# octaviogarcia/RaytracingOneWeekend

Hardware: AMD Instinct MI355X
Metric: Msamples/s (W×H×spp/s) + achieved HBM GB/s, 1080p@512spp traced scene (higher is better)
Workload: dtype f32; 1 GPU; C1 S-traced 1920x1080, 10496 spp timed (128 spp/step), depth 50; width=1920, height=1080, max_depth=50, parallelism=tile1, gather=RCCL send/recv (om_gather_frame), rccl_library=/usr/local/lib/python3.10/dist-packages/torch/lib/librccl.so, kernel=auto, pipeline=auto, tail_bounce=default, streams=2

## Files before the change

raytracingoneweekend_amd/csrc/om_tuning.h:

```cpp
#pragma once

#ifndef OM_WF_BLOCK
#define OM_WF_BLOCK 512
#endif
#ifndef OM_WF_WAVES
#define OM_WF_WAVES 8
#endif
#ifndef OM_WF_TAIL_SPB
#define OM_WF_TAIL_SPB 2
#endif
#ifndef OM_WF_TAIL_WGS_PER_CU
#define OM_WF_TAIL_WGS_PER_CU 1
#endif
#ifndef OM_WF_MAX_PATHS_LOG2
#define OM_WF_MAX_PATHS_LOG2 27
#endif
#ifndef OM_WF_BATCH_SPP
#define OM_WF_BATCH_SPP 16
#endif
#ifndef OM_WF_MIN_PATHS_LOG2
#define OM_WF_MIN_PATHS_LOG2 25
#endif
#ifndef OM_WF_HYB_BYTES
#define OM_WF_HYB_BYTES 16384
#endif
#ifndef OM_WF_HYBW_BYTES
#define OM_WF_HYBW_BYTES 0
#endif
#ifndef OM_WF_HYB4_BYTES
#define OM_WF_HYB4_BYTES 0
#endif
#ifndef OM_WF_REFILL
#define OM_WF_REFILL 16
#endif
#ifndef OM_WF_TAIL_SHADE
#define OM_WF_TAIL_SHADE 1
#endif
#ifndef OM_WF_TAIL_UNROLL
#define OM_WF_TAIL_UNROLL 24
#endif
#ifndef OM_WF_TAIL_MARCH_WAVES
#define OM_WF_TAIL_MARCH_WAVES 8
#endif
#ifndef OM_WF_TAIL_REFILL
#define OM_WF_TAIL_REFILL OM_WF_REFILL
#endif
#ifndef OM_WF_TAIL_MARCHED
#define OM_WF_TAIL_MARCHED 1
#endif
#ifndef OM_MARCH_UNROLL
#define OM_MARCH_UNROLL 8
#endif
#ifndef OM_WF_ADAPTIVE_BATCHES
#define OM_WF_ADAPTIVE_BATCHES 3
#endif
#ifndef OM_WF_ADAPTIVE_PATHS_LOG2
#define OM_WF_ADAPTIVE_PATHS_LOG2 22
#endif
#ifndef OM_WF_ADAPTIVE_CAP_LOG2
#define OM_WF_ADAPTIVE_CAP_LOG2 26
#endif
#ifndef OM_WF_ADAPTIVE_TAIL
#define OM_WF_ADAPTIVE_TAIL 8
#endif
#ifndef OM_WF_LANES_PER_CU
#define OM_WF_LANES_PER_CU 2048
#endif
#ifndef OM_WF_LANES_PER_CU_WIDE
#define OM_WF_LANES_PER_CU_WIDE 8192
#endif
#ifndef OM_WF_DEAL_BLOCKS
#define OM_WF_DEAL_BLOCKS 8
#endif
#ifndef OM_ACC_GROUP
#define OM_ACC_GROUP 8
#endif
#ifndef OM_B2_NODE_STRIDE
#define OM_B2_NODE_STRIDE 80
#endif
#ifndef OM_BARY_TREE_MIN
#define OM_BARY_TREE_MIN 16
#endif
```

raytracingoneweekend_amd/csrc/om_wavefront.hip:

```cpp
#include "om_wavefront.h"

#include <algorithm>
#include <type_traits>

#include "om_device.h"
#include "om_trace.h"
#include "om_tuning.h"
#include "om_deal.h"

using namespace omd;

namespace omw {

void QueueSet::release() {
    for (int a = 0; a < 2; ++a) {
        for (int b = 0; b < 3; ++b) { if (q[a][b]) (void)hipFree(q[a][b]); q[a][b] = nullptr; }
        if (qr[a]) (void)hipFree(qr[a]); qr[a] = nullptr;
    }
    if (res) (void)hipFree(res);
    if (res_id) (void)hipFree(res_id);
    if (counts) (void)hipFree(counts);
    if (hit) (void)hipFree(hit);
    res = nullptr; res_id = nullptr; counts = nullptr; hit = nullptr;
}

void Buffers::release() {
    for (auto& s : set) s.release();
    if (n0) (void)hipFree(n0);
    n0 = nullptr; n0_cap = 0;
    for (auto& st : side) { if (st) (void)hipStreamDestroy(st); st = nullptr; }

    for (auto e : ev) (void)hipEventDestroy(e);
    ev.clear();
    cap = 0; counts_n = 0; nsets = 0;
}

namespace {

constexpr uint32_t kNoSample = 0xFFFFFFFFu;
enum { TR_BRUTE = 1, TR_CULLED = 2, TR_BVH = 3, TR_SBVH_LDS = 4, TR_SBVH_GLOBAL = 5, TR_BVH2_LDS = 6, TR_BVH2_GLOBAL = 7,
       TR_BVH4_LDS = 8, TR_BVH4_GLOBAL = 9,
       TR_BVH2_WIDE = 10,
       TR_BARY = 16 };
constexpr int tr_base(int tr) { return tr & (TR_BARY - 1); }
constexpr bool tr_bary(int tr) { return (tr & TR_BARY) != 0; }
#define OM_WAVES_ATTR __attribute__((amdgpu_waves_per_eu(OM_WF_WAVES, OM_WF_WAVES)))
constexpr int kBlk = OM_WF_BLOCK;
constexpr int kStackDepth = 24;
constexpr uint32_t kB2Stride = OM_B2_NODE_STRIDE;
static_assert(kB2Stride % 16u == 0u && kB2Stride >= sizeof(OmBvh2Node), "16-B aligned node slots");
static_assert(kB2LdsBudget / sizeof(OmBvh2Node) * (kB2Stride / 16u) < OM_LEAF, "scaled BVH2 child codes stay below OM_LEAF");
template <int TR>
__host__ __device__ inline uint32_t stack_bytes(const OmSceneDev& S) {
    if (tr_base(TR) == TR_BVH2_WIDE) return kBlk * S.b2w_stack * 4u;
    return kBlk * ((tr_base(TR) == TR_BVH4_LDS || tr_base(TR) == TR_BVH4_GLOBAL) ? S.b4_stack : S.b2_stack) * 2u;
}
__host__ __device__ inline uint32_t b2_stage_bytes(const OmSceneDev& S) {
    return (S.n_b2nodes * kB2Stride + S.n_b2leaves * 4u + 15u) & ~15u;
}
constexpr uint32_t kTailSpb = OM_WF_TAIL_SPB;
constexpr uint32_t kTailWgsPerCu = OM_WF_TAIL_WGS_PER_CU;
constexpr uint32_t kWaves = kBlk / 64;
static_assert(kBlk % 64 == 0 && kTailWgsPerCu >= 1u, "whole waves; a tail grid");
constexpr uint32_t kTailDefault = 16;
constexpr uint32_t kTailMarched = OM_WF_TAIL_MARCHED;
constexpr uint32_t kTailL2 = 10;
constexpr uint32_t kTailBigBatch = 24;
__host__ __device__ inline uint32_t hyb_nodes(const OmSceneDev& S) {
    constexpr uint32_t kCap = OM_WF_HYB_BYTES / (uint32_t)sizeof(OmBvh2NodeH);
    return S.b2_lds_bytes ? 0u : (S.n_b2nodes < kCap ? S.n_b2nodes : kCap);
}
static_assert(sizeof(OmBvh2NodeW) == sizeof(OmBvh2NodeH), "wide and half nodes share a buffer");
__host__ __device__ inline const OmBvh2NodeW* wide_nodes(const OmSceneDev& S) { return (const OmBvh2NodeW*)(S.b2h + S.n_b2nodes); }
__host__ __device__ inline uint32_t hybw_nodes(const OmSceneDev& S) {
    constexpr uint32_t kCap = OM_WF_HYBW_BYTES / (uint32_t)sizeof(OmBvh2NodeW);
    return S.n_b2wnodes < kCap ? S.n_b2wnodes : kCap;
}
__host__ __device__ inline uint32_t hyb4_nodes(const OmSceneDev& S) {
    constexpr uint32_t kCap = OM_WF_HYB4_BYTES / (uint32_t)sizeof(OmBvh4NodeH);
    return S.b4_lds_bytes ? 0u : (S.n_b4nodes < kCap ? S.n_b4nodes : kCap);
}
using MarchedC2Lds = MarchedExactLds<2, 1, 1>;
enum { MV_ARRAYS = 0, MV_EXACT_C2_LDS = 1 };
template <int TR>
__host__ __device__ constexpr bool exact_view_built() { return TR == TR_BRUTE || TR == TR_BVH2_LDS; }
__host__ __device__ inline Deal batch_deal(uint64_t paths, uint32_t nseg) { return make_deal(paths, nseg, OM_WF_DEAL_BLOCKS); }

extern __shared__ __attribute__((aligned(16))) uint4 wf_lds[];

__device__ __forceinline__ uint32_t wave_sum32(uint32_t v) {
#pragma unroll
    for (int off = 32; off > 0; off >>= 1) v += __shfl_xor(v, off, 64);
    return v;
}
__device__ __forceinline__ void flush_counter(unsigned long long* ctr, int slot, uint32_t v) {
    v = wave_sum32(v);
    if (__lane_id() == 0 && v) atomicAdd(&ctr[slot], (unsigned long long)v);
}

struct Seg {
    uint32_t nseg;
    uint32_t segcap;
};

struct AdPlan { uint32_t c, done; };
struct AdCfg {
    uint32_t sample_count;
    uint32_t batches;
    uint32_t paths;
};
__host__ __device__ inline uint32_t ad_batch(uint32_t c, uint32_t done, uint32_t j, const AdCfg& A) {
    if (c == 0u || done >= A.sample_count || j >= A.batches) return 0u;
    const uint32_t rem = A.sample_count - done, left = A.batches - j;
    const uint32_t even = (rem + left - 1u) / left, want = A.paths / c;
    const uint32_t b = even > want ? even : want;
    return b < rem ? b : rem;
}
struct AdList {
    const uint32_t* list;
    const AdPlan* plan;
    uint32_t* list_next;
    AdPlan* plan_next;
    AdCfg A;
    uint32_t j;
};

struct Queue {
    float4* q0; float4* q1; float4* q2; uint4* qr;
};

struct Gen {
    OmCamDev C;
    const float2* jitter;
    const om_pixel_stats* stats;
    const uint32_t* pixels;
    uint32_t n_pixels, by_pixel, batch;
    const uint32_t* n0;
    uint32_t done;
    AdList ad;
    const uint32_t* tile_off;
    const uint16_t* tile_idx;
    const float* tile_tnear;
};

struct Path {
    F3 o, d, cur;
// ... 123 lines not shown
                                     float& closest, Wk& w) {
    closest = P.tmax;
    int best = trace_traced<TR>(S, T, o, d, P.tmin, closest, w);
    if (MARCH) {
        float tm;
        const int mg = march(S, o, d, P.tmin, P.tmax, closest, P.march_steps, tm, w);
        if (mg >= 0) { best = mg; closest = tm; }
    }
    return best;
}

template <bool MARCH, bool USER = MARCH>
__device__ __forceinline__ bool shade_path(const OmSceneDev& S, const OmParamsDev& P, uint32_t depth_cap, Path& p,
                                           float closest, int best, float4* __restrict__ res,
                                           uint32_t* __restrict__ res_id) {
    float seg_depth; uint32_t seg_id;
    if (best >= 0) {
        F3 point, normal;
        finalize<MARCH, USER>(S, best, p.o, p.d, P.tmin, closest, point, normal);
        F3 nd, att;
        scatter(S.mats[best], p.d, normal, p.g, nd, att);
        p.cur = mul(p.cur, att);
        p.o = point; p.d = unit(nd);
        seg_depth = closest; seg_id = (uint32_t)best + 1u;
    } else {
        const float t = 0.5f * (p.d.y + 1.0f);
        p.cur = mul(p.cur, f3((1.0f - t) + 0.5f * t, (1.0f - t) + 0.7f * t, (1.0f - t) + 1.0f * t));
        seg_depth = INFINITY; seg_id = 0u;
    }
    bool finished = false;
    F3 result = p.cur;
    float rdepth = 0.0f; uint32_t rid = 0;
    if (p.seg == 0u) {
        p.depthf = seg_depth; p.first_id = seg_id;
        if (isinf(seg_depth)) { finished = true; rdepth = INFINITY; rid = 0u; }
    } else if (isinf(seg_depth)) {
        finished = true; rdepth = p.depthf; rid = p.first_id;
    }
    if (!finished && p.seg + 1u >= depth_cap) {
        finished = true; result = f3(-0.0f, -0.0f, -0.0f); rdepth = p.depthf; rid = p.first_id;
    }
    if (finished) {
        res[p.slot] = make_float4(result.x, result.y, result.z, rdepth);
        res_id[p.slot] = rid;
        return false;
    }
    p.seg += 1u;
    return true;
}

__device__ __forceinline__ bool gen_path(const OmParamsDev& P, const Gen& R, uint32_t stride, uint64_t i, Path& p,
                                         uint32_t& pixel, uint32_t* __restrict__ res_id) {
    const uint32_t s_local = (uint32_t)i / stride, kk = (uint32_t)i - s_local * stride;
    const uint32_t k = R.ad.list ? R.ad.list[kk] : kk;
    pixel = R.pixels[k];
    uint32_t s;
    bool live;
    if (R.n0) {
        const uint32_t v = R.n0[k];
        s = (v & 0x7FFFFFFFu) + R.done + s_local;
        live = s < P.spp_total && !(v >> 31);
    } else {
        const om_pixel_stats& ps = R.stats[R.by_pixel ? pixel : k];
        s = ps.n + s_local;
        live = s < P.spp_total && !(P.adaptive && (ps.flags & 1u));
    }
    if (!live) {
        res_id[i] = kNoSample;
        return false;
    }
    p.g = path_rng(P.skey, pixel, s);
    const uint32_t line = pixel / P.width;
    gen_camera_ray(R.C, P, R.jitter, (float)(pixel - P.width * line), (float)line, s, p.g, p.o, p.d);
    p.cur = f3(1.0f, 1.0f, 1.0f); p.depthf = 0.0f; p.first_id = 0u; p.seg = 0u; p.slot = (uint32_t)i;
    return true;
}

template <int TR, bool COUNT, bool MARCH, bool FIRST, bool HIT = false, bool USER = MARCH>
__global__ __launch_bounds__(kBlk) OM_WAVES_ATTR void k_bounce(OmSceneDev S, OmParamsDev P, Seg G, Gen R, Queue in,
                                                 const uint32_t* __restrict__ count_in, Queue out,
                                                 uint32_t* __restrict__ count_out, float4* __restrict__ res,
                                                 uint32_t* __restrict__ res_id, unsigned long long* __restrict__ counters,
                                                 const float2* __restrict__ hitbuf, uint32_t* __restrict__ tail_next) {
    const uint64_t seg0 = (uint64_t)blockIdx.x * G.segcap;
    uint32_t n, stride = R.n_pixels;
    Deal dl{};
    if (FIRST) {
        if (tail_next && blockIdx.x == 0 && threadIdx.x == 0) *tail_next = 0u;
        uint64_t paths = (uint64_t)R.n_pixels * R.batch;
        if (R.ad.list) {
            const AdPlan pl = uniform_load(R.ad.plan);
            stride = pl.c;
            paths = (uint64_t)pl.c * ad_batch(pl.c, pl.done, R.ad.j, R.ad.A);
        }
        dl = batch_deal(paths, G.nseg);
        n = dl.blocks_of(blockIdx.x);
    } else {
        n = count_in[blockIdx.x];
    }
    if (n == 0) {
        if (threadIdx.x == 0) count_out[blockIdx.x] = 0u;
        return;
    }
    __shared__ uint32_t q_next, q_out;
    if (threadIdx.x == 0) { q_next = kBlk / 64u; q_out = 0u; }
    __syncthreads();
    const Tracer T = HIT ? Tracer{} : stage_scene<TR>(S);
    const uint32_t depth_cap = P.max_depth > 1u ? P.max_depth : 1u;
    WorkT<COUNT, false, tr_bary(TR)> w;
    uint32_t segs = 0;
    const uint32_t lane = __lane_id();
    const uint32_t chunks = FIRST ? n : (n + 63u) / 64u;
    for (uint32_t chunk = __builtin_amdgcn_readfirstlane(threadIdx.x >> 6); chunk < chunks;) {
        const uint64_t i = FIRST ? dl.block(blockIdx.x, chunk) * 64u + lane : seg0 + chunk * 64u + lane;
        bool keep = false;
        Path p;
        uint32_t p_pixel = 0;
        if (FIRST ? i < dl.paths : chunk * 64u + lane < n) {
            bool live = true;
            if (FIRST) {
                live = gen_path(P, R, stride, i, p, p_pixel, res_id);
            } else {
                load_ray(in, i, p);
                load_rest(in, i, p);
            }
            if (live) {
                float closest;
                int best;
                if (HIT) {
                    const float2 h = hitbuf[i];
                    closest = h.x; best = __float_as_int(h.y);
                } else if (FIRST && (tr_base(TR) == TR_BVH2_LDS || tr_base(TR) == TR_BVH2_GLOBAL || tr_base(TR) == TR_BVH2_WIDE) && R.tile_off) {
                    const uint32_t line = p_pixel / P.width;
                    const uint32_t tile = (p_pixel - line * P.width) / 8u + (line / 8u) * P.tiles_x;
                    closest = P.tmax;
                    const uint32_t t0 = __builtin_amdgcn_readfirstlane(tile);
                    if (__ballot(tile != t0) == 0)
                        best = traced_tiles<true>(S, R.tile_off, R.tile_idx, t0, p.o, p.d, P.tmin, closest, w, R.tile_tnear);
                    else
                        best = traced_tiles(S, R.tile_off, R.tile_idx, tile, p.o, p.d, P.tmin, closest, w);
                    if (MARCH) {
                        float tm;
                        const int mg = march(S, p.o, p.d, P.tmin, P.tmax, closest, P.march_steps, tm, w);
                        if (mg >= 0) { best = mg; closest = tm; }
                    }
                } else {
                    best = trace<TR, MARCH>(S, P, T, p.o, p.d, closest, w);
                }
                keep = shade_path<MARCH, USER>(S, P, depth_cap, p, closest, best, res, res_id);
                if (COUNT) segs++;
            }
        }
        const uint64_t m = __ballot(keep);
        uint32_t obase = 0u, nc = 0u;
        if (lane == 0) {
            obase = m ? atomicAdd(&q_out, (uint32_t)__popcll(m)) : 0u;
            nc = atomicAdd(&q_next, 1u);
        }
        obase = __builtin_amdgcn_readfirstlane(obase);
        chunk = __builtin_amdgcn_readfirstlane(nc);
        if (keep) store_path(out, seg0 + obase + (uint32_t)__popcll(m & ((1ull << lane) - 1ull)), p);
    }
    __syncthreads();
    if (threadIdx.x == 0) count_out[blockIdx.x] = q_out;
    if (COUNT) {
        flush_counter(counters, OMC_SEGMENTS, segs);
        flush_counter(counters, OMC_PRIM_TESTS, w.prim);
        flush_counter(counters, OMC_PRE_TESTS, w.pre);
        flush_counter(counters, OMC_MARCH, w.march);
    }
}

template <bool COUNT>
__global__ __launch_bounds__(kBlk) OM_WAVES_ATTR void k_raygen(OmParamsDev P, Seg G, Gen R, Queue out,
                                                 uint32_t* __restrict__ count_out, uint32_t* __restrict__ res_id) {
    const uint64_t seg0 = (uint64_t)blockIdx.x * G.segcap;
    uint64_t paths = (uint64_t)R.n_pixels * R.batch;
    uint32_t stride = R.n_pixels;
    if (R.ad.list) {
        const AdPlan pl = uniform_load(R.ad.plan);
        stride = pl.c;
        paths = (uint64_t)pl.c * ad_batch(pl.c, pl.done, R.ad.j, R.ad.A);
    }
    const Deal dl = batch_deal(paths, G.nseg);
    const uint32_t nblk = dl.blocks_of(blockIdx.x);
    __shared__ uint32_t q_out;
    if (threadIdx.x == 0) q_out = 0u;
    __syncthreads();
    const uint32_t lane = __lane_id();
    for (uint32_t c = threadIdx.x >> 6; c < nblk; c += kBlk / 64u) {
        const uint64_t i = dl.block(blockIdx.x, c) * 64u + lane;
        Path p;
        uint32_t pixel;
        const bool keep = i < dl.paths && gen_path(P, R, stride, i, p, pixel, res_id);
        const uint64_t m = __ballot(keep);
        uint32_t obase = 0u;
        if (lane == 0 && m) obase = atomicAdd(&q_out, (uint32_t)__popcll(m));
        obase = __builtin_amdgcn_readfirstlane(obase);
        if (keep) store_path(out, seg0 + obase + (uint32_t)__popcll(m & ((1ull << lane) - 1ull)), p);
    }
    __syncthreads();
    if (threadIdx.x == 0) count_out[blockIdx.x] = q_out;
}

template <int TR, bool COUNT, class M, class Wk>
__device__ __forceinline__ void march_lanes(const OmSceneDev& S, const OmParamsDev& P, const Tracer& T, const M& m,
                                            const Queue& in, uint64_t seg0, uint32_t n, uint32_t& next,
                                            float2* __restrict__ hit, Wk& w) {
    const uint32_t lane = __lane_id();
    uint32_t j = threadIdx.x;
    bool act = j < n, marching = false;
    bool dry = !act;
    F3 o = f3(0.0f, 0.0f, 0.0f), d = o;
    float t = 0.0f, closest = 0.0f;
    int best = -1;
    uint32_t iters = 0;
    auto start = [&]() {
        const float4 a = in.q0[seg0 + j], b = in.q1[seg0 + j];
        o = f3(a.x, a.y, a.z); d = f3(b.x, b.y, b.z);
        best = trace<TR, false>(S, P, T, o, d, closest, w);
        marching = march_begin(m, o, d, P.tmin, t);
        iters = P.march_steps;
    };
    if (act) start();
    for (;;) {
#pragma unroll
        for (int u = 0; u < OM_MARCH_UNROLL; ++u) {
            if (act) {
                int gi = -1;
                const int r = marching ? march_step(S, m, o, d, P.tmax, closest, t, iters, gi, w) : 2;
                if (r != 0) {
                    if (r == 1) { best = gi; closest = t; }
                    hit[seg0 + j] = make_float2(closest, __int_as_float(best));
                    act = false;
                }
            }
        }
        const uint64_t want = __ballot(!act && !dry), busy = __ballot(act);
        if (want && (__popcll(want) >= OM_WF_REFILL || busy == 0)) {
            uint32_t base = 0u;
            if (lane == 0) base = atomicAdd(&next, (uint32_t)__popcll(want));
            base = __builtin_amdgcn_readfirstlane(base);
            if (!act && !dry) {
                j = base + (uint32_t)__popcll(want & ((1ull << lane) - 1ull));
// ... 431 lines not shown
    }
    if (COUNT) {
        flush_counter(counters, OMC_SAMPLES, n_samples);
        flush_counter(counters, OMC_CREDITED, credited);
    }
    if (P.progress) {
        __shared__ unsigned long long wg_credit;
        if (threadIdx.x == 0) wg_credit = 0ull;
        __syncthreads();
        const uint32_t v = wave_sum32(credited);
        if (__lane_id() == 0 && v) atomicAdd(&wg_credit, (unsigned long long)v);
        __syncthreads();
        if (threadIdx.x == 0 && wg_credit) atomicAdd(&counters[OMC_PROGRESS], wg_credit);
    }
}

__global__ __launch_bounds__(256) void k_snapshot(const om_pixel_stats* __restrict__ stats, const uint32_t* __restrict__ pixels,
                                                  uint32_t n_pixels, uint32_t by_pixel, uint32_t* __restrict__ n0) {
    const uint32_t k = blockIdx.x * 256u + threadIdx.x;
    if (k >= n_pixels) return;
    n0[k] = stats[by_pixel ? pixels[k] : k].n;
}

constexpr uint32_t kAdInitBlk = 1024u;
__global__ __launch_bounds__(kAdInitBlk) void k_ad_init(const om_pixel_stats* __restrict__ stats, const uint32_t* __restrict__ pixels,
                                                 uint32_t n_pixels, uint32_t by_pixel, uint32_t spp_total, uint32_t ns,
                                                 uint32_t* __restrict__ lists, uint64_t list_stride, AdPlan* __restrict__ plans,
                                                 uint32_t plan_stride) {
    const uint32_t k = blockIdx.x * kAdInitBlk + threadIdx.x;
    bool live = false;
    if (k < n_pixels) {
        const om_pixel_stats& ps = stats[by_pixel ? pixels[k] : k];
        live = !(ps.flags & 1u) && ps.n < spp_total;
    }
    const uint32_t s = (k >> 6) % ns;
    const uint64_t m = __ballot(live);
    uint32_t base = 0u;
    __shared__ uint32_t wg_n[4], wg_base[4];
    if (threadIdx.x < 4u) wg_n[threadIdx.x] = 0u;
    __syncthreads();
    if (__lane_id() == 0 && m) base = atomicAdd(&wg_n[s], (uint32_t)__popcll(m));
    __syncthreads();
    if (threadIdx.x < ns && wg_n[threadIdx.x])
        wg_base[threadIdx.x] = atomicAdd(&plans[(uint64_t)threadIdx.x * plan_stride].c, wg_n[threadIdx.x]);
    __syncthreads();
    base = __builtin_amdgcn_readfirstlane(base) + (m ? wg_base[s] : 0u);
    if (live) lists[s * list_stride + base + (uint32_t)__popcll(m & ((1ull << __lane_id()) - 1ull))] = k;
}

hipError_t grow(Buffers& B, uint64_t cap, uint32_t counts_n, int nsets) {
    hipError_t e;
    if (cap > B.cap || nsets > B.nsets) {
        for (auto& s : B.set) s.release();
        B.cap = 0; B.nsets = 0; B.counts_n = 0;
        for (int k = 0; k < nsets; ++k) {
            QueueSet& S = B.set[k];
            for (int a = 0; a < 2; ++a) {
                for (int b = 0; b < 3; ++b) if ((e = hipMalloc(&S.q[a][b], cap * sizeof(float4))) != hipSuccess) return e;
                if ((e = hipMalloc(&S.qr[a], cap * sizeof(uint4))) != hipSuccess) return e;
            }
            if ((e = hipMalloc(&S.res, cap * sizeof(float4))) != hipSuccess) return e;
            if ((e = hipMalloc(&S.res_id, cap * sizeof(uint32_t))) != hipSuccess) return e;
            if ((e = hipMalloc(&S.hit, cap * sizeof(float2))) != hipSuccess) return e;
        }
        B.cap = cap; B.nsets = nsets;
    }
    if (counts_n > B.counts_n) {
        for (int k = 0; k < B.nsets; ++k) {
            QueueSet& S = B.set[k];
            if (S.counts) (void)hipFree(S.counts);
            S.counts = nullptr;
            if ((e = hipMalloc(&S.counts, (size_t)counts_n * sizeof(uint32_t))) != hipSuccess) return e;
        }
        B.counts_n = counts_n;
    }
    return hipSuccess;
}

Queue queue(QueueSet& B, int k) { return Queue{B.q[k][0], B.q[k][1], B.q[k][2], B.qr[k]}; }

inline uint32_t tail_pre_off(uint32_t lds) { return (lds + 15u) & ~15u; }
inline uint32_t tail_lds(uint32_t lds, uint32_t nseg) { return tail_pre_off(lds) + (nseg + 1u) * 4u; }

template <int TR, bool COUNT, bool MARCH>
uint32_t run_batch(QueueSet& B, const Launch& L, hipStream_t st, Seg G, const Gen& R, uint32_t depth_cap,
                   uint32_t tail_at, uint32_t lds, uint32_t tail_grid) {
    Timer& tm = *L.timer;
    const bool each = tm.mode == 1;
    uint32_t launches = 0;
    const bool exact = MARCH && L.S.n_msdf == 0u && MarchedC2Lds::matches(L.S.n_msph, L.S.n_mbox, L.S.n_mtor);
    uint32_t* const tail_next = B.counts + (size_t)(depth_cap + 1u) * G.nseg;
    auto tail = [&](const Queue& in, const uint32_t* cin) {
        const int ti = each ? tm.begin(st) : -1;
        if constexpr (MARCH) {
            const uint32_t grid = (G.nseg + kTailSpb - 1u) / kTailSpb;
            if (exact && exact_view_built<TR>())
                hipLaunchKernelGGL((k_tail_march<TR, COUNT, exact_view_built<TR>() ? MV_EXACT_C2_LDS : MV_ARRAYS>), dim3(grid),
                                   dim3(kBlk), lds, st, L.S, L.P, G, in, cin, B.res, B.res_id, L.counters);
            else
                hipLaunchKernelGGL((k_tail_march<TR, COUNT>), dim3(grid), dim3(kBlk), lds, st, L.S, L.P, G, in, cin,
                                   B.res, B.res_id, L.counters);
        } else {
            hipLaunchKernelGGL((k_tail<TR, COUNT>), dim3(tail_grid), dim3(kBlk), tail_lds(lds, G.nseg), st, L.S, L.P, G, in, cin,
                               tail_pre_off(lds), tail_next, B.res, B.res_id, L.counters);
        }
        tm.end(ti, OM_KT_TAIL, st);
        return launches + 1u;
    };
    if constexpr (MARCH) {
        {
            const int ti = each ? tm.begin(st) : -1;
            hipLaunchKernelGGL((k_raygen<COUNT>), dim3(G.nseg), dim3(kBlk), 0, st, L.P, G, R, queue(B, 0), B.counts, B.res_id);
            tm.end(ti, OM_KT_BOUNCE0, st);
            ++launches;
        }
        for (uint32_t bounce = 0; bounce < depth_cap; ++bounce) {
            const Queue in = queue(B, bounce & 1u), out = queue(B, (bounce + 1u) & 1u);
            const uint32_t* cin = B.counts + (size_t)bounce * G.nseg;
            if (bounce >= tail_at) return tail(in, cin);
            uint32_t* cout = B.counts + (size_t)(bounce + 1u) * G.nseg;
            const int kc = bounce == 0 ? OM_KT_BOUNCE0 : OM_KT_BOUNCE;
            int ti = each ? tm.begin(st) : -1;
            if (exact && exact_view_built<TR>())
                hipLaunchKernelGGL((k_march<TR, COUNT, exact_view_built<TR>() ? MV_EXACT_C2_LDS : MV_ARRAYS>), dim3(G.nseg),
                                   dim3(kBlk), lds, st, L.S, L.P, G, in, cin, B.hit, L.counters);
            else
                hipLaunchKernelGGL((k_march<TR, COUNT, MV_ARRAYS>), dim3(G.nseg), dim3(kBlk), lds, st, L.S, L.P, G, in, cin,
                                   B.hit, L.counters);
            tm.end(ti, kc, st);
            ti = each ? tm.begin(st) : -1;
            if (exact && exact_view_built<TR>())
                hipLaunchKernelGGL((k_bounce<TR, COUNT, MARCH, false, true, false>), dim3(G.nseg), dim3(kBlk), 0, st, L.S, L.P, G,
                                   R, in, cin, out, cout, B.res, B.res_id, L.counters, (const float2*)B.hit, (uint32_t*)nullptr);
            else
                hipLaunchKernelGGL((k_bounce<TR, COUNT, MARCH, false, true>), dim3(G.nseg), dim3(kBlk), 0, st, L.S, L.P, G, R, in,
                                   cin, out, cout, B.res, B.res_id, L.counters, (const float2*)B.hit, (uint32_t*)nullptr);
            tm.end(ti, kc, st);
            launches += 2u;
        }
        return launches;
    } else {
    for (uint32_t bounce = 0; bounce < depth_cap; ++bounce) {
        const Queue in = queue(B, bounce & 1u), out = queue(B, (bounce + 1u) & 1u);
        const uint32_t* cin = B.counts + (size_t)bounce * G.nseg;
        if (bounce > 0 && bounce >= tail_at) return tail(in, cin);
        uint32_t* cout = B.counts + (size_t)(bounce + 1u) * G.nseg;
        const int ti = each ? tm.begin(st) : -1;
        if (bounce == 0)
            hipLaunchKernelGGL((k_bounce<TR, COUNT, MARCH, true>), dim3(G.nseg), dim3(kBlk), lds, st, L.S, L.P, G, R, in,
                               cin, out, cout, B.res, B.res_id, L.counters, (const float2*)nullptr, tail_next);
        else
            hipLaunchKernelGGL((k_bounce<TR, COUNT, MARCH, false>), dim3(G.nseg), dim3(kBlk), lds, st, L.S, L.P, G, R, in,
                               cin, out, cout, B.res, B.res_id, L.counters, (const float2*)nullptr, (uint32_t*)nullptr);
        tm.end(ti, bounce == 0 ? OM_KT_BOUNCE0 : OM_KT_BOUNCE, st);
        ++launches;
    }
    return launches;
    }
}

template <int TR>
uint32_t run_tr(bool count, bool march, QueueSet& B, const Launch& L, hipStream_t st, Seg G, const Gen& R,
                uint32_t depth_cap, uint32_t tail_at, uint32_t lds, uint32_t tail_grid) {
    if (count && march) return run_batch<TR, true, true>(B, L, st, G, R, depth_cap, tail_at, lds, tail_grid);
    if (count) return run_batch<TR, true, false>(B, L, st, G, R, depth_cap, tail_at, lds, tail_grid);
    if (march) return run_batch<TR, false, true>(B, L, st, G, R, depth_cap, tail_at, lds, tail_grid);
    return run_batch<TR, false, false>(B, L, st, G, R, depth_cap, tail_at, lds, tail_grid);
}

hipError_t ensure_events(Buffers& B, size_t n) {
    while (B.ev.size() < n) {
        hipEvent_t e = nullptr;
        const hipError_t r = hipEventCreateWithFlags(&e, hipEventDisableTiming);
        if (r != hipSuccess) return r;
        B.ev.push_back(e);
    }
    return hipSuccess;
}

int pick_trace(int trace_mode, const OmSceneDev& S) {
    int tr = trace_mode == TR_SBVH_LDS ? TR_SBVH_GLOBAL : trace_mode;
    if (tr == TR_BVH2_WIDE) {
        if (S.n_b2wnodes) return TR_BVH2_WIDE | TR_BARY;
        tr = TR_BVH2_LDS;
    }
    if (tr == TR_BVH4_LDS) tr = S.n_b4nodes == 0 ? TR_BVH2_LDS : (S.b4_lds_bytes ? TR_BVH4_LDS : TR_BVH4_GLOBAL);
    if (tr == TR_BVH2_LDS && S.n_b2nodes == 0 && S.n_b2wnodes) return TR_BVH2_WIDE | TR_BARY;
    if (tr == TR_BVH2_LDS)
        tr = S.n_b2nodes == 0 ? (S.n_bvh_nodes <= 1u ? TR_BRUTE : TR_BVH) : (S.b2_lds_bytes ? TR_BVH2_LDS : TR_BVH2_GLOBAL);
    const int bary = S.n_srec_bary ? TR_BARY : 0;
    switch (tr) {
        case TR_BRUTE: case TR_CULLED: case TR_BVH: return tr;
        case TR_SBVH_GLOBAL: case TR_BVH2_LDS: case TR_BVH4_LDS: case TR_BVH4_GLOBAL: return tr | bary;
        default: return TR_BVH2_GLOBAL | bary;
    }
}
uint32_t trace_lds(int trf, const OmSceneDev& S) {
    const int tr = tr_base(trf);
    return tr == TR_BVH2_LDS ? stack_bytes<TR_BVH2_LDS>(S) + b2_stage_bytes(S)
         : tr == TR_BVH2_GLOBAL ? stack_bytes<TR_BVH2_GLOBAL>(S) + hyb_nodes(S) * (uint32_t)sizeof(OmBvh2NodeH)
         : tr == TR_BVH4_LDS ? stack_bytes<TR_BVH4_LDS>(S) + S.b4_lds_bytes
         : tr == TR_BVH4_GLOBAL ? stack_bytes<TR_BVH4_GLOBAL>(S) + hyb4_nodes(S) * (uint32_t)sizeof(OmBvh4NodeH)
         : tr == TR_BVH2_WIDE ? stack_bytes<TR_BVH2_WIDE>(S) + hybw_nodes(S) * (uint32_t)sizeof(OmBvh2NodeW)
         : 0u;
}
template <class F>
void with_tr(int tr, F f) {
    switch (tr) {
        case TR_BRUTE: f(std::integral_constant<int, TR_BRUTE>{}); break;
        case TR_CULLED: f(std::integral_constant<int, TR_CULLED>{}); break;
        case TR_BVH: f(std::integral_constant<int, TR_BVH>{}); break;
        case TR_SBVH_GLOBAL: f(std::integral_constant<int, TR_SBVH_GLOBAL>{}); break;
        case TR_BVH2_LDS: f(std::integral_constant<int, TR_BVH2_LDS>{}); break;
        case TR_BVH4_LDS: f(std::integral_constant<int, TR_BVH4_LDS>{}); break;
        case TR_BVH4_GLOBAL: f(std::integral_constant<int, TR_BVH4_GLOBAL>{}); break;
        case TR_SBVH_GLOBAL | TR_BARY: f(std::integral_constant<int, TR_SBVH_GLOBAL | TR_BARY>{}); break;
        case TR_BVH2_LDS | TR_BARY: f(std::integral_constant<int, TR_BVH2_LDS | TR_BARY>{}); break;
        case TR_BVH2_GLOBAL | TR_BARY: f(std::integral_constant<int, TR_BVH2_GLOBAL | TR_BARY>{}); break;
        case TR_BVH4_LDS | TR_BARY: f(std::integral_constant<int, TR_BVH4_LDS | TR_BARY>{}); break;
        case TR_BVH4_GLOBAL | TR_BARY: f(std::integral_constant<int, TR_BVH4_GLOBAL | TR_BARY>{}); break;
        case TR_BVH2_WIDE | TR_BARY: f(std::integral_constant<int, TR_BVH2_WIDE | TR_BARY>{}); break;
        default: f(std::integral_constant<int, TR_BVH2_GLOBAL>{}); break;
    }
}

template <int TR, bool MARCH, bool USER>
void launch_query(const Query& Q, const OmParamsDev& P, uint32_t grid, uint32_t lds, hipStream_t st) {
    if (Q.windows) {
        if (Q.count)
            hipLaunchKernelGGL((k_query_windows<TR, MARCH, USER, true>), dim3(grid), dim3(kBlk), lds, st, Q.S, P, Q.rays, Q.windows, Q.n, Q.hits, Q.counters);
        else
            hipLaunchKernelGGL((k_query_windows<TR, MARCH, USER, false>), dim3(grid), dim3(kBlk), lds, st, Q.S, P, Q.rays, Q.windows, Q.n, Q.hits, Q.counters);
    } else if (Q.count)
        hipLaunchKernelGGL((k_query<TR, MARCH, USER, true>), dim3(grid), dim3(kBlk), lds, st, Q.S, P, Q.rays, Q.n, Q.hits, Q.counters);
    else
        hipLaunchKernelGGL((k_query<TR, MARCH, USER, false>), dim3(grid), dim3(kBlk), lds, st, Q.S, P, Q.rays, Q.n, Q.hits, Q.counters);
}
template <int TR, bool MARCH>
void launch_occluded(const Query& Q, const OmParamsDev& P, uint32_t grid, uint32_t lds, hipStream_t st) {
    if (Q.count)
        hipLaunchKernelGGL((k_occluded<TR, MARCH, true>), dim3(grid), dim3(kBlk), lds, st, Q.S, P, Q.rays, Q.windows, Q.n, Q.occluded, Q.counters);
    else
        hipLaunchKernelGGL((k_occluded<TR, MARCH, false>), dim3(grid), dim3(kBlk), lds, st, Q.S, P, Q.rays, Q.windows, Q.n, Q.occluded, Q.counters);
}

}

hipError_t render(Buffers& B, const Launch& L, hipStream_t st, std::string& err) {
    const uint32_t n_px = L.n_pixels;
    if (n_px == 0 || L.P.sample_count == 0) return hipSuccess;
    const bool adaptive = L.P.adaptive != 0u;
    const uint32_t want = std::max<uint32_t>(1u, std::min<uint32_t>(L.streams, (uint32_t)kMaxSets));
    const uint64_t kMaxPaths = std::min<uint64_t>(1ull << OM_WF_MAX_PATHS_LOG2,
                                                  std::max<uint64_t>(1ull << OM_WF_MIN_PATHS_LOG2, (uint64_t)OM_WF_BATCH_SPP * n_px));
    uint32_t ns, nb, batch = 0, ad_k = 0, cmax = 0;
    uint64_t max_paths;
    std::vector<uint32_t> done_at(1, 0u);
    AdCfg A{};
    if (adaptive) {
        const uint32_t chunks = (n_px + 63u) / 64u;
        ns = std::min<uint32_t>(want, chunks);
        cmax = std::min<uint32_t>(n_px, (chunks + ns - 1u) / ns * 64u);
        const uint64_t capmax = 1ull << OM_WF_ADAPTIVE_CAP_LOG2;
        uint64_t k = L.ad_batches ? L.ad_batches : OM_WF_ADAPTIVE_BATCHES;
        while (k < L.P.sample_count && (uint64_t)cmax * ((L.P.sample_count + k - 1u) / k) > capmax) ++k;
        ad_k = (uint32_t)std::min<uint64_t>(k, L.P.sample_count);
        A.sample_count = L.P.sample_count; A.batches = ad_k;
        A.paths = 1u << (L.ad_paths_log2 ? L.ad_paths_log2 : OM_WF_ADAPTIVE_PATHS_LOG2);
        max_paths = std::max<uint64_t>(std::min<uint64_t>(A.paths, (uint64_t)cmax * L.P.sample_count),
                                       (uint64_t)cmax * ((L.P.sample_count + ad_k - 1u) / ad_k));
        nb = ad_k * ns;
    } else {
        const bool concurrent = want >= 2u && L.P.sample_count >= 2u;
        batch = (uint32_t)std::max<uint64_t>(1, std::min<uint64_t>(L.P.sample_count, kMaxPaths / n_px));
        if (concurrent) batch = std::min<uint32_t>(batch, (L.P.sample_count + want - 1u) / want);
        while (done_at.back() < L.P.sample_count)
            done_at.push_back(done_at.back() + std::min(batch, L.P.sample_count - done_at.back()));
        nb = (uint32_t)done_at.size() - 1u;
        ns = concurrent ? std::min<uint32_t>(want, nb) : 1u;
        max_paths = (uint64_t)n_px * batch;
    }
    const uint32_t depth_cap = L.P.max_depth > 1u ? L.P.max_depth : 1u;
    int dev = 0;
    (void)hipGetDevice(&dev);
    int cus = 256;
    (void)hipDeviceGetAttribute(&cus, hipDeviceAttributeMultiprocessorCount, dev);
    const int tr = pick_trace(L.trace_mode, L.S);
    const bool march = (L.S.n_msph + L.S.n_mbox + L.S.n_mtor + L.S.n_msdf) != 0u;
    const bool l2_tree = tr_base(tr) == TR_BVH2_GLOBAL || tr_base(tr) == TR_BVH4_GLOBAL || tr_base(tr) == TR_BVH2_WIDE;
    const uint32_t tail_at = L.tail_bounce ? L.tail_bounce
                           : march ? kTailMarched : l2_tree ? kTailL2
                           : adaptive ? OM_WF_ADAPTIVE_TAIL
                           : max_paths > (1ull << 25) ? kTailBigBatch : kTailDefault;
    const uint32_t lanes_per_cu = (march || l2_tree) ? OM_WF_LANES_PER_CU_WIDE : OM_WF_LANES_PER_CU;
    const uint32_t nseg = deal_segments(max_paths, (uint32_t)cus, lanes_per_cu, kBlk, kTailSpb);
    const uint32_t segcap = batch_deal(max_paths, nseg).capacity();
    hipError_t e = grow(B, (uint64_t)nseg * segcap, (depth_cap + 1u) * nseg + 1u, (int)ns);
    if (e != hipSuccess) { err = "wavefront buffer allocation failed"; return e; }
    const uint32_t lds = trace_lds(tr, L.S);
    const uint32_t tail_grid = (uint32_t)cus * kTailWgsPerCu;
    int lds_max = 0;
    (void)hipDeviceGetAttribute(&lds_max, hipDeviceAttributeMaxSharedMemoryPerBlock, dev);
    if (!march && tail_at < depth_cap && tail_lds(lds, nseg) > (uint32_t)lds_max) {
        err = "the tail's LDS request exceeds the device's limit";
        return hipErrorInvalidValue;
    }
    if (lds > (uint32_t)lds_max) {
        err = "the traversal's LDS request exceeds the device's limit";
        return hipErrorInvalidValue;
    }
    Gen R;
    R.C = L.C; R.jitter = L.jitter; R.stats = L.stats; R.pixels = L.pixels; R.n_pixels = n_px;
    R.by_pixel = L.stats_by_pixel ? 1u : 0u;
    R.tile_off = L.tile_off; R.tile_idx = L.tile_idx; R.tile_tnear = L.tile_tnear;
    R.n0 = nullptr; R.done = 0; R.ad = AdList{};
    hipStream_t streams[kMaxSets] = {st, st, st, st};
    Timer& tm = *L.timer;
    const int call_ti = tm.begin(st);
    const uint32_t plan_stride = ad_k + 1u;
    const uint64_t words = adaptive ? (uint64_t)ns * 2u * cmax + (uint64_t)ns * plan_stride * 2u : (ns > 1 ? n_px : 0u);
    if (words > B.n0_cap) {
        if (B.n0) (void)hipFree(B.n0);
        B.n0 = nullptr; B.n0_cap = 0;
        if ((e = hipMalloc(&B.n0, (size_t)words * sizeof(uint32_t))) != hipSuccess) { err = "n0 allocation failed"; return e; }
        B.n0_cap = words;
    }
    uint32_t* lists = B.n0;
    AdPlan* plans = adaptive ? (AdPlan*)(B.n0 + (uint64_t)ns * 2u * cmax) : nullptr;
    if (adaptive) {
        (void)hipMemsetAsync(plans, 0, (size_t)ns * plan_stride * sizeof(AdPlan), st);
        hipLaunchKernelGGL(k_ad_init, dim3((n_px + kAdInitBlk - 1u) / kAdInitBlk), dim3(kAdInitBlk), 0, st, L.stats, L.pixels, n_px, R.by_pixel,
                           L.P.spp_total, ns, lists, (uint64_t)2u * cmax, plans, plan_stride);
    } else if (ns > 1) {
        hipLaunchKernelGGL(k_snapshot, dim3((n_px + 255u) / 256u), dim3(256), 0, st, L.stats, L.pixels, n_px, R.by_pixel, B.n0);
        R.n0 = B.n0;
    }
    if (ns > 1) {
        if ((e = ensure_events(B, kMaxSets + nb)) != hipSuccess) { err = "event creation failed"; return e; }
        (void)hipEventRecord(B.ev[0], st);
        for (uint32_t k = 1; k < ns; ++k) {
            if (!B.side[k] && (e = hipStreamCreateWithFlags(&B.side[k], hipStreamNonBlocking)) != hipSuccess) {
                err = "side stream creation failed"; return e;
            }
            streams[k] = B.side[k];
            (void)hipStreamWaitEvent(streams[k], B.ev[0], 0);
        }
    }
    uint32_t launches = 0;
    for (uint32_t i = 0; i < nb; ++i) {
        const uint32_t sidx = i % ns;
        hipStream_t si = streams[sidx];
        QueueSet& QS = B.set[sidx];
        Seg G;
        G.nseg = nseg;
        uint32_t b = 0, grid_a;
        AdList ad{};
        if (adaptive) {
            const uint32_t j = i / ns;
            uint32_t* lbase = lists + (uint64_t)sidx * 2u * cmax;
            ad.list = lbase + (uint64_t)(j & 1u) * cmax;
            ad.list_next = lbase + (uint64_t)((j + 1u) & 1u) * cmax;
            ad.plan = plans + (uint64_t)sidx * plan_stride + j;
            ad.plan_next = plans + (uint64_t)sidx * plan_stride + j + 1u;
            ad.A = A; ad.j = j;
            G.segcap = segcap;
            grid_a = (cmax + kBlk - 1) / kBlk;
        } else {
            const uint32_t done = done_at[i];
            b = done_at[i + 1] - done;
            G.segcap = batch_deal((uint64_t)n_px * b, nseg).capacity();
            R.done = done;
            grid_a = (n_px + kBlk - 1) / kBlk;
        }
        R.batch = b;
        R.ad = ad;
        with_tr(tr, [&](auto t) {
            launches += run_tr<decltype(t)::value>(L.count, march, QS, L, si, G, R, depth_cap, tail_at, lds, tail_grid);
        });
        if (ns > 1 && i > 0) (void)hipStreamWaitEvent(si, B.ev[kMaxSets + i - 1u], 0);
        const int ati = tm.mode == 1 ? tm.begin(si) : -1;
// ... 67 lines not shown
```

Measured before the change: 7646 Msamples/s.

## Fuse first two bounces into one wavefront kernel launch

The first-bounce kernel now traces and shades a second bounce in-register for non-marched scenes, skipping one queue store/load round trip and one kernel launch. Bounce scheduling advances by two after bounce 0, the count buffer gains an extra row, and the tail threshold shifts by one to keep the same tail point. It also swaps the popcount prefix for mbcnt intrinsics and forces the stride into a scalar register. The cost is higher register pressure and more divergence in the first kernel, since lanes whose path ended sit idle during the second bounce.

```diff
diff --git a/raytracingoneweekend_amd/csrc/om_tuning.h b/raytracingoneweekend_amd/csrc/om_tuning.h
--- a/raytracingoneweekend_amd/csrc/om_tuning.h
+++ b/raytracingoneweekend_amd/csrc/om_tuning.h
@@ -72,6 +72,9 @@
 #ifndef OM_WF_DEAL_BLOCKS
 #define OM_WF_DEAL_BLOCKS 8
 #endif
+#ifndef OM_WF_FUSE_B1
+#define OM_WF_FUSE_B1 1
+#endif
 #ifndef OM_ACC_GROUP
 #define OM_ACC_GROUP 8
 #endif
diff --git a/raytracingoneweekend_amd/csrc/om_wavefront.hip b/raytracingoneweekend_amd/csrc/om_wavefront.hip
--- a/raytracingoneweekend_amd/csrc/om_wavefront.hip
+++ b/raytracingoneweekend_amd/csrc/om_wavefront.hip
@@ -62,6 +62,7 @@
 constexpr uint32_t kTailWgsPerCu = OM_WF_TAIL_WGS_PER_CU;
 constexpr uint32_t kWaves = kBlk / 64;
 static_assert(kBlk % 64 == 0 && kTailWgsPerCu >= 1u, "whole waves; a tail grid");
+constexpr bool kFuseB1 = OM_WF_FUSE_B1 != 0;
 constexpr uint32_t kTailDefault = 16;
 constexpr uint32_t kTailMarched = OM_WF_TAIL_MARCHED;
 constexpr uint32_t kTailL2 = 10;
@@ -351,6 +352,7 @@
                                                  uint32_t* __restrict__ count_out, float4* __restrict__ res,
                                                  uint32_t* __restrict__ res_id, unsigned long long* __restrict__ counters,
                                                  const float2* __restrict__ hitbuf, uint32_t* __restrict__ tail_next) {
+    constexpr bool FUSE = FIRST && !MARCH && !HIT && kFuseB1;
     const uint64_t seg0 = (uint64_t)blockIdx.x * G.segcap;
     uint32_t n, stride = R.n_pixels;
     Deal dl{};
@@ -381,44 +383,53 @@
     const uint32_t lane = __lane_id();
     const uint32_t chunks = FIRST ? n : (n + 63u) / 64u;
     for (uint32_t chunk = __builtin_amdgcn_readfirstlane(threadIdx.x >> 6); chunk < chunks;) {
-        const uint64_t i = FIRST ? dl.block(blockIdx.x, chunk) * 64u + lane : seg0 + chunk * 64u + lane;
+        const uint64_t i = FUSE  ? (uint64_t)((uint32_t)(dl.block(blockIdx.x, chunk) * 64u) + lane)
+                         : FIRST ? dl.block(blockIdx.x, chunk) * 64u + lane : seg0 + chunk * 64u + lane;
         bool keep = false;
         Path p;
         uint32_t p_pixel = 0;
         if (FIRST ? i < dl.paths : chunk * 64u + lane < n) {
-            bool live = true;
             if (FIRST) {
-                live = gen_path(P, R, stride, i, p, p_pixel, res_id);
+                uint32_t st = stride;
+                if (FUSE) asm volatile("" : "+s"(st));
+                keep = gen_path(P, R, st, i, p, p_pixel, res_id);
             } else {
                 load_ray(in, i, p);
                 load_rest(in, i, p);
+                keep = true;
             }
-            if (live) {
-                float closest;
-                int best;
+        }
+        float closest = 0.0f;
+        int best = -1;
+        const bool listed = FIRST && !HIT && (tr_base(TR) == TR_BVH2_LDS || tr_base(TR) == TR_BVH2_GLOBAL || tr_base(TR) == TR_BVH2_WIDE) && R.tile_off;
+        if (listed && keep) {
+            const uint32_t line = p_pixel / P.width;
+            const uint32_t tile = (p_pixel - line * P.width) / 8u + (line / 8u) * P.tiles_x;
+            closest = P.tmax;
+            const uint32_t t0 = __builtin_amdgcn_readfirstlane(tile);
+            if (__ballot(tile != t0) == 0)
+                best = traced_tiles<true>(S, R.tile_off, R.tile_idx, t0, p.o, p.d, P.tmin, closest, w, R.tile_tnear);
+            else
+                best = traced_tiles(S, R.tile_off, R.tile_idx, tile, p.o, p.d, P.tmin, closest, w);
+            if (MARCH) {
+                float tm;
+                const int mg = march(S, p.o, p.d, P.tmin, P.tmax, closest, P.march_steps, tm, w);
+                if (mg >= 0) { best = mg; closest = tm; }
+            }
+        }
+#pragma clang loop unroll(disable)
+        for (uint32_t sg = 0u;; ++sg) {
+            if (keep) {
                 if (HIT) {
                     const float2 h = hitbuf[i];
                     closest = h.x; best = __float_as_int(h.y);
-                } else if (FIRST && (tr_base(TR) == TR_BVH2_LDS || tr_base(TR) == TR_BVH2_GLOBAL || tr_base(TR) == TR_BVH2_WIDE) && R.tile_off) {
-                    const uint32_t line = p_pixel / P.width;
-                    const uint32_t tile = (p_pixel - line * P.width) / 8u + (line / 8u) * P.tiles_x;
-                    closest = P.tmax;
-                    const uint32_t t0 = __builtin_amdgcn_readfirstlane(tile);
-                    if (__ballot(tile != t0) == 0)
-                        best = traced_tiles<true>(S, R.tile_off, R.tile_idx, t0, p.o, p.d, P.tmin, closest, w, R.tile_tnear);
-                    else
-                        best = traced_tiles(S, R.tile_off, R.tile_idx, tile, p.o, p.d, P.tmin, closest, w);
-                    if (MARCH) {
-                        float tm;
-                        const int mg = march(S, p.o, p.d, P.tmin, P.tmax, closest, P.march_steps, tm, w);
-                        if (mg >= 0) { best = mg; closest = tm; }
-                    }
-                } else {
+                } else if (!(listed && sg == 0u)) {
                     best = trace<TR, MARCH>(S, P, T, p.o, p.d, closest, w);
                 }
                 keep = shade_path<MARCH, USER>(S, P, depth_cap, p, closest, best, res, res_id);
                 if (COUNT) segs++;
             }
+            if (!FUSE || sg == 1u || __ballot(keep) == 0) break;
         }
         const uint64_t m = __ballot(keep);
         uint32_t obase = 0u, nc = 0u;
@@ -428,7 +439,9 @@
         }
         obase = __builtin_amdgcn_readfirstlane(obase);
         chunk = __builtin_amdgcn_readfirstlane(nc);
-        if (keep) store_path(out, seg0 + obase + (uint32_t)__popcll(m & ((1ull << lane) - 1ull)), p);
+        const uint32_t rank = FUSE ? __builtin_amdgcn_mbcnt_hi((uint32_t)(m >> 32), __builtin_amdgcn_mbcnt_lo((uint32_t)m, 0u))
+                                   : (uint32_t)__popcll(m & ((1ull << lane) - 1ull));
+        if (keep) store_path(out, seg0 + obase + rank, p);
     }
     __syncthreads();
     if (threadIdx.x == 0) count_out[blockIdx.x] = q_out;
@@ -1026,6 +1039,8 @@
 inline uint32_t tail_pre_off(uint32_t lds) { return (lds + 15u) & ~15u; }
 inline uint32_t tail_lds(uint32_t lds, uint32_t nseg) { return tail_pre_off(lds) + (nseg + 1u) * 4u; }
 
+inline uint32_t count_rows(uint32_t depth_cap) { return std::max<uint32_t>(depth_cap, kFuseB1 ? 2u : 1u) + 1u; }
+
 template <int TR, bool COUNT, bool MARCH>
 uint32_t run_batch(QueueSet& B, const Launch& L, hipStream_t st, Seg G, const Gen& R, uint32_t depth_cap,
                    uint32_t tail_at, uint32_t lds, uint32_t tail_grid) {
@@ -1033,7 +1048,7 @@
     const bool each = tm.mode == 1;
     uint32_t launches = 0;
     const bool exact = MARCH && L.S.n_msdf == 0u && MarchedC2Lds::matches(L.S.n_msph, L.S.n_mbox, L.S.n_mtor);
-    uint32_t* const tail_next = B.counts + (size_t)(depth_cap + 1u) * G.nseg;
+    uint32_t* const tail_next = B.counts + (size_t)count_rows(depth_cap) * G.nseg;
     auto tail = [&](const Queue& in, const uint32_t* cin) {
         const int ti = each ? tm.begin(st) : -1;
         if constexpr (MARCH) {
@@ -1084,11 +1099,12 @@
         }
         return launches;
     } else {
-    for (uint32_t bounce = 0; bounce < depth_cap; ++bounce) {
-        const Queue in = queue(B, bounce & 1u), out = queue(B, (bounce + 1u) & 1u);
+    for (uint32_t bounce = 0, next; bounce < depth_cap; bounce = next) {
+        next = bounce + (bounce == 0 && kFuseB1 ? 2u : 1u);
+        const Queue in = queue(B, bounce & 1u), out = queue(B, next & 1u);
         const uint32_t* cin = B.counts + (size_t)bounce * G.nseg;
         if (bounce > 0 && bounce >= tail_at) return tail(in, cin);
-        uint32_t* cout = B.counts + (size_t)(bounce + 1u) * G.nseg;
+        uint32_t* cout = B.counts + (size_t)next * G.nseg;
         const int ti = each ? tm.begin(st) : -1;
         if (bounce == 0)
             hipLaunchKernelGGL((k_bounce<TR, COUNT, MARCH, true>), dim3(G.nseg), dim3(kBlk), lds, st, L.S, L.P, G, R, in,
@@ -1233,13 +1249,13 @@
     const bool march = (L.S.n_msph + L.S.n_mbox + L.S.n_mtor + L.S.n_msdf) != 0u;
     const bool l2_tree = tr_base(tr) == TR_BVH2_GLOBAL || tr_base(tr) == TR_BVH4_GLOBAL || tr_base(tr) == TR_BVH2_WIDE;
     const uint32_t tail_at = L.tail_bounce ? L.tail_bounce
-                           : march ? kTailMarched : l2_tree ? kTailL2
-                           : adaptive ? OM_WF_ADAPTIVE_TAIL
-                           : max_paths > (1ull << 25) ? kTailBigBatch : kTailDefault;
+                           : march ? kTailMarched
+                           : (l2_tree ? kTailL2 : adaptive ? OM_WF_ADAPTIVE_TAIL
+                              : max_paths > (1ull << 25) ? kTailBigBatch : kTailDefault) + (kFuseB1 ? 1u : 0u);
     const uint32_t lanes_per_cu = (march || l2_tree) ? OM_WF_LANES_PER_CU_WIDE : OM_WF_LANES_PER_CU;
     const uint32_t nseg = deal_segments(max_paths, (uint32_t)cus, lanes_per_cu, kBlk, kTailSpb);
     const uint32_t segcap = batch_deal(max_paths, nseg).capacity();
-    hipError_t e = grow(B, (uint64_t)nseg * segcap, (depth_cap + 1u) * nseg + 1u, (int)ns);
+    hipError_t e = grow(B, (uint64_t)nseg * segcap, count_rows(depth_cap) * nseg + 1u, (int)ns);
     if (e != hipSuccess) { err = "wavefront buffer allocation failed"; return e; }
     const uint32_t lds = trace_lds(tr, L.S);
     const uint32_t tail_grid = (uint32_t)cus * kTailWgsPerCu;
```

Measured after the change: 8091 Msamples/s, median of 6. 5.8% higher.
